# a1q123456/image_stitching

Measured on AMD Instinct MI355X. Metric: 4K frames stitched/sec, higher is better.
Workload: dtype u8

## Files before the change

image_stitching_amd/csrc/orb.hip:

```cpp
#include "common.h"
#include "dev_math.h"
#include <algorithm>
#include <cmath>
#include <mutex>
#include <unordered_map>

#define ORB_MAX_LEVELS 16
#define ORB_BORDER 32

namespace {

struct LevelDesc {
    int w, h;
    int pp;
    int sp;
    size_t pad_off;
    size_t map_off;
    float scale;
    int nfeat;
    int n2;
    int tiles_x, tiles_y, tile_off;
    int cap1, cand_off;
    int cap2, fin_off;
    int tab_off;
};

struct Levels {
    int n;
    int fast_t, patch, half_patch, edge;
    LevelDesc d[ORB_MAX_LEVELS];
};

struct Work {
    uint8_t *pad, *blur, *score, *nms;
    int* hist;
    int* thr;
    int* tile_cnt;
    uint32_t* surv_xy;
    uint8_t* surv_sc;
    int* cnt1;
    int* cnt2;
    int* flags;
    uint32_t* cand_xy;
    float* cand_resp;
    uint32_t* fin_xy;
    float* fin_resp;
    int* tab;
    int* umax;
    int8_t* pattern;
};

constexpr int ORB_BATCH = 16;
struct OrbIO {
    const uint8_t* src[ORB_BATCH];
    size_t sstride[ORB_BATCH];
    int aligned[ORB_BATCH];
    MisKeyPoint* kps[ORB_BATCH];
    uint32_t* lxy[ORB_BATCH];
    int* n_dev[ORB_BATCH];
    uint8_t* desc[ORB_BATCH];
// ... 157 lines not shown
    if ((px & 3) == 0) *reinterpret_cast<unsigned*>(p + ro + px) = v;
    else
#pragma unroll
        for (int k = 0; k < 4; k++) p[ro + px + k] = (uint8_t)(v >> (8 * k));
}

__device__ __forceinline__ bool fast_pretest(const uint8_t* p, int pp, int t) {
    const int v = p[0], hi = v + t, lo = v - t;
    const int c0 = p[3 * pp], c4 = p[3], c8 = p[-3 * pp], c12 = p[-3];
    unsigned br = (c0 > hi) | ((c4 > hi) << 2) | ((c8 > hi) << 4) | ((c12 > hi) << 6);
    unsigned dk = (c0 < lo) | ((c4 < lo) << 2) | ((c8 < lo) << 4) | ((c12 < lo) << 6);
    const unsigned adj_b = br & ((br >> 2) | (br << 6)), adj_d = dk & ((dk >> 2) | (dk << 6));
    if (!((adj_b | adj_d) & 0x55)) return false;
    const int c2 = p[2 * pp + 2], c6 = p[-2 * pp + 2], c10 = p[-2 * pp - 2], c14 = p[2 * pp - 2];
    br |= ((c2 > hi) << 1) | ((c6 > hi) << 3) | ((c10 > hi) << 5) | ((c14 > hi) << 7);
    dk |= ((c2 < lo) << 1) | ((c6 < lo) << 3) | ((c10 < lo) << 5) | ((c14 < lo) << 7);
    const unsigned b2 = br | (br << 8), d2 = dk | (dk << 8);
    const unsigned rb = b2 & (b2 >> 1) & (b2 >> 2) & (b2 >> 3), rd = d2 & (d2 >> 1) & (d2 >> 2) & (d2 >> 3);
    return ((rb | rd) & 0xff) != 0;
}
__device__ __forceinline__ int fast_score_full(const uint8_t* p, int pp, int t) {
    const int v = p[0];
    int d[16];
    d[0] = v - p[3 * pp]; d[1] = v - p[3 * pp + 1]; d[2] = v - p[2 * pp + 2]; d[3] = v - p[pp + 3];
    d[4] = v - p[3]; d[5] = v - p[-pp + 3]; d[6] = v - p[-2 * pp + 2]; d[7] = v - p[-3 * pp + 1];
    d[8] = v - p[-3 * pp]; d[9] = v - p[-3 * pp - 1]; d[10] = v - p[-2 * pp - 2]; d[11] = v - p[-pp - 3];
    d[12] = v - p[-3]; d[13] = v - p[pp - 3]; d[14] = v - p[2 * pp - 2]; d[15] = v - p[3 * pp - 1];
    int n3[16], x3[16];
#pragma unroll
    for (int i = 0; i < 16; i++) {
        n3[i] = min(min(d[i], d[(i + 1) & 15]), d[(i + 2) & 15]);
        x3[i] = max(max(d[i], d[(i + 1) & 15]), d[(i + 2) & 15]);
    }
    int A = -512, Bm = 512;
#pragma unroll
    for (int i = 0; i < 16; i++) {
        A = max(A, min(min(n3[i], n3[(i + 3) & 15]), n3[(i + 6) & 15]));
        Bm = min(Bm, max(max(x3[i], x3[(i + 3) & 15]), x3[(i + 6) & 15]));
    }
    const int best = max(A, -Bm);
    return best > t ? best - 1 : 0;
}
__device__ __forceinline__ int fast_score_px(const uint8_t* p, int pp, int t) { return fast_pretest(p, pp, t) ? fast_score_full(p, pp, t) : 0; }

#ifndef MIS_FT_ROWS
#define MIS_FT_ROWS 64
#endif
constexpr int FT_COLS = 64, FT_ROWS = MIS_FT_ROWS, FG_PITCH = 96, FG_COL0 = 15, HIST_COPIES = 8;
constexpr int FT_WR = (FT_ROWS + 2 + 3) / 4;
constexpr int FT_SLOTS = FT_COLS * FT_ROWS / 4;
#ifdef MIS_ORB_STATS
__device__ unsigned long long g_orb_stats[8];
#endif
__global__ __launch_bounds__(256) void fast_nms_kernel(Levels L, const uint8_t* pad, int* hist, int* tile_cnt, uint32_t* surv_xy, uint8_t* surv_sc, size_t ws) {
    __shared__ __attribute__((aligned(16))) uint8_t g[(FT_ROWS + 10) * FG_PITCH];
    __shared__ __attribute__((aligned(16))) uint8_t sc[(FT_ROWS + 2) * (FT_COLS + 4)];
    __shared__ int lh[256];
    __shared__ int lcount;
    __shared__ uint32_t lxy[FT_SLOTS];
    __shared__ uint8_t lsc[FT_SLOTS];
    __shared__ unsigned short queue[(FT_ROWS + 2) * (FT_COLS + 2)];
    __shared__ int qcount;
    const int fz = blockIdx.z / L.n, lz = blockIdx.z - fz * L.n;
    const LevelDesc& d = L.d[lz];
    const int x0 = blockIdx.x * FT_COLS, y0 = blockIdx.y * FT_ROWS, t = threadIdx.x;
    if (x0 >= d.w || y0 >= d.h) return;
    WS_OFF(pad, fz, ws); WS_OFF(hist, fz, ws); WS_OFF(tile_cnt, fz, ws); WS_OFF(surv_xy, fz, ws); WS_OFF(surv_sc, fz, ws);
    lh[t] = 0;
    if (t == 0) { lcount = 0; qcount = 0; }
    {
        const int ph = d.h + 2 * ORB_BORDER;
        const uint8_t* src = pad + d.pad_off;
        const int px0 = x0 - 16 + ORB_BORDER, py0 = y0 - 4 + ORB_BORDER;
        for (int i = t; i < (FT_ROWS + 8) * (FG_PITCH / 16); i += 256) {
            const int r = i / (FG_PITCH / 16), c = i - r * (FG_PITCH / 16);
            const int py = min(py0 + r, ph - 1);
            int px = px0 + 16 * c;
            if (px + 15 >= d.pp) px = d.pp - 16;
            reinterpret_cast<uint4*>(g)[i] = *reinterpret_cast<const uint4*>(src + (size_t)py * d.pp + px);
        }
    }
    __syncthreads();
    const int SP = FT_COLS + 4;
    for (int i = t; i < (FT_ROWS + 2) * SP / 4; i += 256) reinterpret_cast<unsigned*>(sc)[i] = 0u;
    {
        const int wv = __builtin_amdgcn_readfirstlane(t >> 6), lane = t & 63;
        const unsigned ft = (unsigned)L.fast_t;
        const int r0 = FT_WR * wv;
        bool pass[FT_WR + 1];
        unsigned long long ball[FT_WR + 1];
        int total = 0;
        {
            const uint8_t* colp = g + r0 * FG_PITCH + (lane + FG_COL0);
            unsigned col[FT_WR + 6];
#pragma unroll
            for (int j = 0; j < FT_WR + 6; j++) col[j] = colp[j * FG_PITCH];
            const int x = x0 - 1 + lane;
            const bool xin = x >= 3 && x < d.w - 3;
            const uint8_t* rowp = g + (r0 + 3) * FG_PITCH + (lane + FG_COL0 - 3);
#pragma unroll
            for (int k = 0; k < FT_WR; k++) {
                const int r = r0 + k, y = y0 - 1 + r;
                const bool rowok = r < FT_ROWS + 2 && y >= 3 && y < d.h - 3;
                const unsigned v = col[k + 3];
                const unsigned dv = max(__builtin_amdgcn_sad_u8(col[k + 6], v, 0u), __builtin_amdgcn_sad_u8(col[k], v, 0u));
                const unsigned dh = max(__builtin_amdgcn_sad_u8(rowp[k * FG_PITCH + 6], v, 0u), __builtin_amdgcn_sad_u8(rowp[k * FG_PITCH], v, 0u));
                pass[k] = rowok & xin & (min(dv, dh) > ft);
                ball[k] = __ballot(pass[k]);
                total += __popcll(ball[k]);
            }
        }
        {
            const int k = lane >> 1, cc = FT_COLS + (lane & 1), r = r0 + k, y = y0 - 1 + r, x = x0 - 1 + cc;
            bool ps = false;
            if (lane < 2 * FT_WR && r < FT_ROWS + 2) {
                const uint8_t* pp = g + (r + 3) * FG_PITCH + (cc + FG_COL0);
// ... 16 lines not shown
                const int r = k < FT_WR ? r0 + k : r0 + (lane >> 1), c = k < FT_WR ? lane : FT_COLS + (lane & 1);
                queue[base + __popcll(ball[k] & below)] = (unsigned short)(r * (FT_COLS + 2) + c);
            }
            base += __popcll(ball[k]);
        }
    }
    __syncthreads();
    for (int q = t; q < qcount; q += 256) {
        const int i = queue[q], r = i / (FT_COLS + 2), c = i - r * (FT_COLS + 2);
        const int fsv = fast_score_full(g + (r + 3) * FG_PITCH + (c + FG_COL0), FG_PITCH, L.fast_t);
        sc[r * SP + c] = (uint8_t)fsv;
#ifdef MIS_ORB_STATS
        if (fsv) atomicAdd(&g_orb_stats[3], 1ull);
#endif
    }
    __syncthreads();
    {
        const int nq = qcount;
        for (int q0 = 0; q0 < nq; q0 += 256) {
            const int q = q0 + t;
            bool keep = false;
            int x = 0, y = 0, v = 0;
            if (q < nq) {
                const int i = queue[q], r = i / (FT_COLS + 2), c = i - r * (FT_COLS + 2);
                const uint8_t* s_ = sc + r * SP + c;
                v = s_[0];
                x = x0 - 1 + c; y = y0 - 1 + r;
                keep = v && r >= 1 && r <= FT_ROWS && c >= 1 && c <= FT_COLS && x >= L.edge && x < d.w - L.edge && y >= L.edge && y < d.h - L.edge &&
                       v > s_[-1] && v > s_[1] && v > s_[-SP - 1] && v > s_[-SP] && v > s_[-SP + 1] && v > s_[SP - 1] && v > s_[SP] && v > s_[SP + 1];
            }
            const unsigned long long m = __ballot(keep);
            int base = 0;
            if ((t & 63) == 0 && m) base = atomicAdd(&lcount, __popcll(m));
            base = __shfl(base, 0);
            if (keep) {
                const int j = base + __popcll(m & ((1ull << (t & 63)) - 1ull));
                lxy[j] = (uint32_t)x | ((uint32_t)y << 16); lsc[j] = (uint8_t)v;
            }
        }
    }
    __syncthreads();
    const int n = lcount;
    const int tile = d.tile_off + blockIdx.y * d.tiles_x + blockIdx.x;
    if (t == 0) tile_cnt[tile] = n;
    if (n == 0) return;
    for (int j = t; j < n; j += 256) {
        atomicAdd(&lh[lsc[j]], 1);
        surv_xy[(size_t)tile * FT_SLOTS + j] = lxy[j]; surv_sc[(size_t)tile * FT_SLOTS + j] = lsc[j];
    }
    __syncthreads();
    if (lh[t]) atomicAdd(&hist[((lz * HIST_COPIES) + ((blockIdx.x + blockIdx.y) & (HIST_COPIES - 1))) * 256 + t], lh[t]);
}

__global__ __launch_bounds__(256) void fast_cut_kernel(Levels L, const int* hist, int* thr, int* flags, size_t ws) {
    __shared__ int suf[256];
    __shared__ int s_thr;
    const int l = blockIdx.x, t = threadIdx.x;
    WS_OFF(hist, blockIdx.y, ws); WS_OFF(thr, blockIdx.y, ws); WS_OFF(flags, blockIdx.y, ws);
    const LevelDesc& d = L.d[l];
    int hsum = 0;
    for (int c = 0; c < HIST_COPIES; c++) hsum += hist[(l * HIST_COPIES + c) * 256 + t];
    suf[t] = t ? hsum : 0;
    __syncthreads();
    for (int o = 1; o < 256; o <<= 1) {
        int add = t + o < 256 ? suf[t + o] : 0;
        __syncthreads();
        suf[t] += add;
        __syncthreads();
    }
    if (t == 0) s_thr = d.n2 == 0 ? 256 : 1;
    __syncthreads();
    if (d.n2 > 0 && suf[1] > d.n2 && t >= 1 && suf[t] >= d.n2 && (t == 255 || suf[t + 1] < d.n2)) s_thr = t;
    __syncthreads();
    if (t == 0) {
        thr[l] = s_thr;
        if (s_thr < 256 && suf[s_thr] > d.cap1) atomicOr(&flags[0], 1);
    }
}

constexpr int CT_TILES = 16;
__global__ __launch_bounds__(256) void compact_kernel(Levels L, const int* tile_cnt, const uint32_t* surv_xy, const uint8_t* surv_sc, const int* thr,
                                                      int* cnt1, uint32_t* cand_xy, float* cand_resp, size_t ws) {
    __shared__ int s_cnt[CT_TILES], s_off[CT_TILES];
    __shared__ int s_base;
    const int l = blockIdx.y, t = threadIdx.x, lane = t & 63, wave = t >> 6;
    WS_OFF(tile_cnt, blockIdx.z, ws); WS_OFF(surv_xy, blockIdx.z, ws); WS_OFF(surv_sc, blockIdx.z, ws); WS_OFF(thr, blockIdx.z, ws);
    WS_OFF(cnt1, blockIdx.z, ws); WS_OFF(cand_xy, blockIdx.z, ws); WS_OFF(cand_resp, blockIdx.z, ws);
    const LevelDesc& d = L.d[l];
    const int ntiles = d.tiles_x * d.tiles_y, first = blockIdx.x * CT_TILES;
    if (first >= ntiles) return;
    const int th = thr[l];
    for (int k = 0; k < CT_TILES / 4; k++) {
        const int slot = wave * (CT_TILES / 4) + k, til = first + slot;
        int cnt = 0;
        if (til < ntiles) {
            const int tile = d.tile_off + til, n = tile_cnt[tile];
            for (int j0 = 0; j0 < n; j0 += 64) {
                const int j = j0 + lane;
                const int v = j < n ? surv_sc[(size_t)tile * FT_SLOTS + j] : 0;
                cnt += __popcll(__ballot(v >= th && v > 0));
            }
        }
        if (lane == 0) s_cnt[slot] = cnt;
    }
    __syncthreads();
    if (t == 0) {
        int tot = 0;
        for (int k = 0; k < CT_TILES; k++) { s_off[k] = tot; tot += s_cnt[k]; }
        s_base = tot ? atomicAdd(&cnt1[l], tot) : 0;
    }
    __syncthreads();
    for (int k = 0; k < CT_TILES / 4; k++) {
        const int slot = wave * (CT_TILES / 4) + k, til = first + slot;
        if (til >= ntiles || s_cnt[slot] == 0) continue;
        const int tile = d.tile_off + til, n = tile_cnt[tile];
        int run = s_base + s_off[slot];
        for (int j0 = 0; j0 < n; j0 += 64) {
            const int j = j0 + lane;
            const int v = j < n ? surv_sc[(size_t)tile * FT_SLOTS + j] : 0;
            const bool keep = v >= th && v > 0;
            const unsigned long long m = __ballot(keep);
            if (keep) {
                const int i = run + __popcll(m & ((1ull << lane) - 1ull));
                if (i < d.cap1) { cand_xy[d.cand_off + i] = surv_xy[(size_t)tile * FT_SLOTS + j]; cand_resp[d.cand_off + i] = (float)v; }
            }
            run += __popcll(m);
        }
    }
}

__global__ void nms_raster_kernel(LevelDesc d, const int* tile_cnt, const uint32_t* surv_xy, const uint8_t* surv_sc, uint8_t* nms) {
    const int ntiles = d.tiles_x * d.tiles_y;
    for (int tl = blockIdx.x; tl < ntiles; tl += gridDim.x) {
        const int tile = d.tile_off + tl, n = tile_cnt[tile];
        for (int j = threadIdx.x; j < n; j += blockDim.x) {
            uint32_t xy = surv_xy[(size_t)tile * FT_SLOTS + j];
            nms[d.map_off + (size_t)(xy >> 16) * d.sp + (xy & 0xffff)] = surv_sc[(size_t)tile * FT_SLOTS + j];
        }
    }
}

__global__ __launch_bounds__(256) void harris_kernel(Levels L, const uint8_t* pad, const int* cnt1, const uint32_t* cand_xy, float* cand_resp, size_t ws) {
    const LevelDesc& d = L.d[blockIdx.y];
    WS_OFF(pad, blockIdx.z, ws); WS_OFF(cnt1, blockIdx.z, ws); WS_OFF(cand_xy, blockIdx.z, ws); WS_OFF(cand_resp, blockIdx.z, ws);
    int i = blockIdx.x * 256 + threadIdx.x;
    int n = min(cnt1[blockIdx.y], d.cap1);
    if (i >= n) return;
    uint32_t xy = cand_xy[d.cand_off + i];
    int x = xy & 0xffff, y = xy >> 16;
    const int pp = d.pp;
    const uint8_t* q0 = pad + d.pad_off + (size_t)(y + ORB_BORDER - 4) * pp + (x + ORB_BORDER - 4);
    const unsigned sh = (unsigned)((uintptr_t)q0 & 3u);
    const uint8_t* a0 = q0 - sh;
    int px[9][9];
#pragma unroll
    for (int r = 0; r < 9; r++) {
        const unsigned* row = reinterpret_cast<const unsigned*>(a0 + (size_t)r * pp);
        const unsigned d0 = row[0], d1 = row[1], d2 = row[2];
        const unsigned w0 = __builtin_amdgcn_alignbyte(d1, d0, sh), w1 = __builtin_amdgcn_alignbyte(d2, d1, sh), w2 = __builtin_amdgcn_alignbyte(0u, d2, sh);
#pragma unroll
        for (int k = 0; k < 4; k++) { px[r][k] = (int)((w0 >> (8 * k)) & 255u); px[r][4 + k] = (int)((w1 >> (8 * k)) & 255u); }
        px[r][8] = (int)(w2 & 255u);
    }
    int a = 0, b = 0, c = 0;
#pragma unroll
    for (int by = 0; by < 7; by++)
#pragma unroll
        for (int bx = 0; bx < 7; bx++) {
            const int Ix = (px[by + 1][bx + 2] - px[by + 1][bx]) * 2 + (px[by][bx + 2] - px[by][bx]) + (px[by + 2][bx + 2] - px[by + 2][bx]);
            const int Iy = (px[by + 2][bx + 1] - px[by][bx + 1]) * 2 + (px[by + 2][bx] - px[by][bx]) + (px[by + 2][bx + 2] - px[by][bx + 2]);
            a += Ix * Ix; b += Iy * Iy; c += Ix * Iy;
        }
    const float scale = 1.f / ((1 << 2) * 7 * 255.f);
    const float scale_sq_sq = scale * scale * scale * scale;
    float fa = (float)a, fb = (float)b, fc = (float)c;
    float s1 = fa * fb, s2 = fc * fc;
    float s3 = 0.04f * (fa + fb);
    s3 = s3 * (fa + fb);
    cand_resp[d.cand_off + i] = ((s1 - s2) - s3) * scale_sq_sq;
}

__device__ __forceinline__ uint32_t fkey(float f) {
    uint32_t u = __float_as_uint(f);
    return (u & 0x80000000u) ? ~u : (u | 0x80000000u);
}

__global__ __launch_bounds__(1024) void select_rank_kernel(Levels L, const int* cnt1, const uint32_t* cand_xy, const float* cand_resp,
                                                            int* cnt2, uint32_t* fin_xy, float* fin_resp, int* flags, int use_harris, size_t ws) {
    WS_OFF(cnt1, blockIdx.y, ws); WS_OFF(cand_xy, blockIdx.y, ws); WS_OFF(cand_resp, blockIdx.y, ws); WS_OFF(cnt2, blockIdx.y, ws);
    WS_OFF(fin_xy, blockIdx.y, ws); WS_OFF(fin_resp, blockIdx.y, ws); WS_OFF(flags, blockIdx.y, ws);
    __shared__ int hist[256];
    __shared__ uint32_t s_prefix, s_mask;
    __shared__ int s_k, s_m;
    __shared__ uint32_t kkey[4096], kxy[4096];
    const int l = blockIdx.x, t = threadIdx.x;
    const LevelDesc& d = L.d[l];
    const int n = min(cnt1[l], d.cap1);
    const uint32_t* xy = cand_xy + d.cand_off;
    const float* rs = cand_resp + d.cand_off;
    const int N = d.nfeat;
    if (N == 0) { if (t == 0) cnt2[l] = 0; return; }
    if (n <= 4096) {
        int P = 1;
        while (P < n) P <<= 1;
        for (int i = t; i < P; i += 1024) {
            if (i < n) { kkey[i] = fkey(rs[i]); kxy[i] = xy[i]; }
            else { kkey[i] = 0; kxy[i] = 0xffffffffu; }
        }
        __syncthreads();
        for (int k = 2; k <= P; k <<= 1)
            for (int j = k >> 1; j > 0; j >>= 1) {
                for (int i = t; i < P; i += 1024) {
                    const int ixj = i ^ j;
                    if (ixj > i) {
                        const uint32_t ka = kkey[i], kb = kkey[ixj], pa = kxy[i], pb = kxy[ixj];
                        const bool a_first = ka > kb || (ka == kb && pa < pb);
                        const bool descending_block = (i & k) == 0;
                        if (a_first != descending_block) { kkey[i] = kb; kkey[ixj] = ka; kxy[i] = pb; kxy[ixj] = pa; }
                    }
                }
                __syncthreads();
            }
        const uint32_t cutk = (use_harris && n > N) ? kkey[N - 1] : 0u;
        if (t == 0) s_m = 0;
        __syncthreads();
        for (int i = t; i < n; i += 1024)
            if (kkey[i] >= cutk && (i == n - 1 || kkey[i + 1] < cutk)) s_m = i + 1;
        __syncthreads();
        const int m = s_m;
        if (m > d.cap2) { if (t == 0) { atomicOr(&flags[0], 2); cnt2[l] = 0; } return; }
        for (int i = t; i < m; i += 1024) {
            fin_xy[d.fin_off + i] = kxy[i];
            const uint32_t ki = kkey[i], uu = (ki & 0x80000000u) ? (ki & 0x7fffffffu) : ~ki;
            fin_resp[d.fin_off + i] = __uint_as_float(uu);
        }
        if (t == 0) cnt2[l] = m;
        return;
    }
    uint32_t cut = 0;
    if (use_harris && n > N) {
        if (t == 0) { s_prefix = 0; s_mask = 0; s_k = N; }
        __syncthreads();
        for (int shift = 24; shift >= 0; shift -= 8) {
            if (t < 256) hist[t] = 0;
            __syncthreads();
            uint32_t prefix = s_prefix, mask = s_mask;
            for (int i = t; i < n; i += 1024) {
                uint32_t k = fkey(rs[i]);
// ... 266 lines not shown
        for (int j = 0; j < 7; j++) {
            const unsigned d0 = q[j * (DD_PITCH / 4)], d1 = q[j * (DD_PITCH / 4) + 1], d2 = q[j * (DD_PITCH / 4) + 2];
            const unsigned lo = __builtin_amdgcn_alignbit(d1, d0, sh), hi = __builtin_amdgcn_alignbit(d2, d1, sh);
            const unsigned hs = __builtin_amdgcn_udot4(lo, 0x38302212u, __builtin_amdgcn_udot4(hi, 0x00122230u, 0u, false), false);
            acc += (unsigned)kq[j] * hs;
            if (j == 3) centre = lo >> 24;
        }
        return inside ? (int)((acc + (1u << 15)) >> 16) : (int)centre;
    };
    int val = 0;
#ifndef DD_UNROLL
#define DD_UNROLL 1
#endif
#pragma unroll DD_UNROLL
    for (int bit = 0; bit < 4; bit++) {
        float x0 = (float)pat[4 * bit], y0 = (float)pat[4 * bit + 1], x1 = (float)pat[4 * bit + 2], y1 = (float)pat[4 * bit + 3];
        int ix0 = mis_round_f(x0 * ca - y0 * sa), iy0 = mis_round_f(x0 * sa + y0 * ca);
        int ix1 = mis_round_f(x1 * ca - y1 * sa), iy1 = mis_round_f(x1 * sa + y1 * ca);
        const int t0 = blurred(ix0, iy0), t1 = blurred(ix1, iy1);
        val |= (t0 < t1) << (bit + 4 * h);
    }
    val |= __shfl_xor(val, 32);
    if (h == 0) desc[(size_t)i * 32 + b] = (uint8_t)val;
}

constexpr int ORB_GATHER_MAX = 96;
struct GatherPtrs { const int* p[ORB_GATHER_MAX]; };
__global__ void gather_ints_kernel(GatherPtrs g, int n, int* __restrict__ out) {
    const int i = blockIdx.x * blockDim.x + threadIdx.x;
    if (i < n) out[i] = *g.p[i];
}

}

struct MisOrb {
    MisContext* ctx = nullptr;
    void (*enqueued_cb)(void*) = nullptr;
    void* enqueued_user = nullptr;
    MisOrbParams p;
    int max_w = 0, max_h = 0;
    int cur_w = 0, cur_h = 0;
    Levels L;
    Work w;
    size_t ws_stride = 0;
    int ws_frames = 0;
    int umax_host[64] = {0};
    int8_t pattern_host[1024] = {0};
    void* mem = nullptr;
    size_t pad_bytes = 0, map_bytes = 0;
    int cand_total = 0, fin_total = 0, tab_total = 0, surv_total = 0, out_cap = 0;
    std::vector<int> tab_host;
    int* host_counts = nullptr;
    bool direct_describe = false;
};

namespace {

void linear_exact_coeffs(int dlen, int slen, int* ofs, int* m1) {
    double inv = (double)dlen / (double)slen, scale = 1.0 / inv;
    for (int i = 0; i < dlen; i++) {
        double v = ((double)i + 0.5) * scale - 0.5;
        int iv = (int)floor(v);
        if (iv < 0) { ofs[i] = 0; m1[i] = 0; }
        else if (iv >= slen - 1) { ofs[i] = slen - 1; m1[i] = 0; }
        else { ofs[i] = iv; m1[i] = (int)lrint((v - (double)iv) * 256.0); }
    }
}

constexpr int ORB_MAX_LEVEL_FEATURES = 2048 - 128;

inline float level_scale(const MisOrbParams& p, int l) { return (float)pow((double)p.scale_factor, (double)l); }
inline int level_dim(int len, float sc) { return (int)lrint((double)((float)len / sc)); }

void level_budgets(const MisOrbParams& p, int* nfeat) {
    float factor = (float)(1.0 / (double)p.scale_factor);
    float nd = (float)p.nfeatures * (1 - factor) / (1 - (float)pow((double)factor, (double)p.nlevels));
    int sum = 0;
    for (int l = 0; l < p.nlevels - 1; l++) { nfeat[l] = (int)lrintf(nd); sum += nfeat[l]; nd *= factor; }
    nfeat[p.nlevels - 1] = std::max(p.nfeatures - sum, 0);
}

int check_level_sizes(MisContext* ctx, const MisOrbParams& p, int w, int h) {
    for (int l = 0; l < p.nlevels; l++) {
        const float sc = level_scale(p, l);
        MIS_CHECK(ctx, level_dim(w, sc) >= 1 && level_dim(h, sc) >= 1, MIS_E_UNSUPPORTED,
                  "ORB level %d of a %dx%d frame is empty (scale_factor %g, nlevels %d)", l, w, h, (double)p.scale_factor, p.nlevels);
    }
    return MIS_OK;
}

void plan_levels(MisOrb* o, int w, int h) {
    Levels& L = o->L;
    const MisOrbParams& p = o->p;
    L.n = p.nlevels; L.fast_t = p.fast_threshold; L.patch = p.patch_size; L.half_patch = p.patch_size / 2; L.edge = p.edge_threshold;
    size_t pad_off = 0, map_off = 0;
    int cand_off = 0, fin_off = 0, tab_off = 0, surv_off = 0;
    int nfeat[ORB_MAX_LEVELS];
    level_budgets(p, nfeat);
    for (int l = 0; l < L.n; l++) {
        LevelDesc& d = L.d[l];
        float sc = level_scale(p, l);
        d.scale = sc;
        d.w = level_dim(w, sc);
        d.h = level_dim(h, sc);
        d.pp = (int)mis_align_up((size_t)d.w + 2 * ORB_BORDER, 64);
        d.sp = (int)mis_align_up((size_t)d.w, 64);
// ... 7 lines not shown
        d.cap2 = std::min(d.nfeat + 128, 2048);
        d.cand_off = cand_off; cand_off += d.cap1;
        d.fin_off = fin_off; fin_off += d.cap2;
        d.tab_off = tab_off; tab_off += (2 * ((d.w + 3) & ~3) + 2 * d.h + 3) & ~3;
    }
    o->pad_bytes = pad_off; o->map_bytes = map_off; o->cand_total = cand_off; o->fin_total = fin_off; o->tab_total = tab_off; o->surv_total = surv_off;
    o->tab_host.assign(tab_off, 0);
    for (int l = 1; l < L.n; l++) {
        int* t = o->tab_host.data() + L.d[l].tab_off;
        const int dw4 = (L.d[l].w + 3) & ~3;
        linear_exact_coeffs(L.d[l].w, L.d[l - 1].w, t, t + dw4);
        linear_exact_coeffs(L.d[l].h, L.d[l - 1].h, t + 2 * dw4, t + 2 * dw4 + L.d[l].h);
    }
}

int upload_tables(MisOrb* o) {
    MisContext* ctx = o->ctx;
    if (o->tab_total)
        MIS_HIP(ctx, hipMemcpyAsync(o->w.tab, o->tab_host.data(), sizeof(int) * o->tab_total, hipMemcpyHostToDevice, ctx->stream));
    MIS_HIP(ctx, hipStreamSynchronize(ctx->stream));
    return MIS_OK;
}

std::mutex g_feat_mutex;
std::unordered_map<void*, size_t> g_feat_sizes;

int alloc_features(MisContext* ctx, int cap, int desc_cols, int desc_dtype, MisFeatures* f) {
    size_t kb = mis_align_up(sizeof(MisKeyPoint) * (size_t)cap, 256), db = mis_align_up((size_t)cap * desc_cols * mis_dtype_size(desc_dtype), 256);
    size_t lb = mis_align_up(sizeof(uint32_t) * (size_t)cap, 256);
    void* mem = nullptr;
    size_t got = 0;
    int rc = mis_pool_alloc(ctx, kb + db + lb + 256, &mem, &got);
    if (rc != MIS_OK) return rc;
    f->keypoints = (MisKeyPoint*)mem;
    f->descriptors = (uint8_t*)mem + kb;
    f->desc_cols = desc_cols; f->desc_dtype = desc_dtype;
    f->owner_ = mem;
    f->n = 0;
    std::lock_guard<std::mutex> lock(g_feat_mutex);
    g_feat_sizes[mem] = got;
    return MIS_OK;
}

inline uint32_t* feat_lxy(const MisFeatures* f, int cap) {
    size_t kb = mis_align_up(sizeof(MisKeyPoint) * (size_t)cap, 256), db = mis_align_up((size_t)cap * f->desc_cols * mis_dtype_size(f->desc_dtype), 256);
    return (uint32_t*)((uint8_t*)f->owner_ + kb + db);
}
inline int* feat_count(const MisFeatures* f, int cap) {
    size_t kb = mis_align_up(sizeof(MisKeyPoint) * (size_t)cap, 256), db = mis_align_up((size_t)cap * f->desc_cols * mis_dtype_size(f->desc_dtype), 256);
    size_t lb = mis_align_up(sizeof(uint32_t) * (size_t)cap, 256);
    return (int*)((uint8_t*)f->owner_ + kb + db + lb);
}

int enqueue_detect_group(MisOrb* o, const DevView* img, int w, int h, MisFeatures* out, int ng) {
    MisContext* ctx = o->ctx;
    const Levels& L = o->L;
    const Work& W = o->w;
    hipStream_t st = ctx->stream;
    const LevelDesc& d0 = L.d[0];
    const size_t ws = o->ws_stride;
    const unsigned nf = (unsigned)ng;
    OrbIO io;
    for (int k = 0; k < ORB_BATCH; k++) {
        const int q = k < ng ? k : 0;
        io.src[k] = (const uint8_t*)img[q].data; io.sstride[k] = img[q].stride;
        io.aligned[k] = (img[q].stride % 4 == 0) && ((uintptr_t)img[q].data % 4 == 0);
        io.kps[k] = out[q].keypoints; io.lxy[k] = feat_lxy(&out[q], o->out_cap); io.n_dev[k] = feat_count(&out[q], o->out_cap);
        io.desc[k] = (uint8_t*)out[q].descriptors;
    }
    MIS_HIP(ctx, hipMemset2DAsync(W.hist, ws ? ws : sizeof(int) * (256 * HIST_COPIES * ORB_MAX_LEVELS + 4 * ORB_MAX_LEVELS), 0,
                                  sizeof(int) * (256 * HIST_COPIES * ORB_MAX_LEVELS + 4 * ORB_MAX_LEVELS), nf, st));
    hipLaunchKernelGGL(gray_kernel, dim3((w + 1023) / 1024, (h + GRAY_ROWS - 1) / GRAY_ROWS, nf), dim3(256), 0, st, io, w, h, W.pad + d0.pad_off, d0.pp, ws);
    for (int l = 1; l < L.n; l++) {
        const LevelDesc &s = L.d[l - 1], &d = L.d[l];
        hipLaunchKernelGGL(resize_kernel, dim3((d.w + 255) / 256, (d.h + 4 * RS_ROWS - 1) / (4 * RS_ROWS), nf), dim3(256), 0, st, W.pad + s.pad_off, s.w, s.h, s.pp, W.pad + d.pad_off, d.w,
                           d.h, d.pp, W.tab + d.tab_off, ws);
    }
    const int pw0 = d0.w + 2 * ORB_BORDER, ph0 = d0.h + 2 * ORB_BORDER;
    hipLaunchKernelGGL((border_kernel<true>), dim3((d0.h * 16 + 255) / 256, 1, L.n * nf), dim3(256), 0, st, L, W.pad, ws);
    hipLaunchKernelGGL((border_kernel<false>), dim3((pw0 + 1023) / 1024, 2 * ORB_BORDER / 4, L.n * nf), dim3(256), 0, st, L, W.pad, ws);
    dim3 gmap((d0.w + FT_COLS - 1) / FT_COLS, (d0.h + FT_ROWS - 1) / FT_ROWS, L.n * nf);
    hipLaunchKernelGGL(fast_nms_kernel, gmap, dim3(256), 0, st, L, W.pad, W.hist, W.tile_cnt, W.surv_xy, W.surv_sc, ws);
    hipLaunchKernelGGL(fast_cut_kernel, dim3(L.n, nf), dim3(256), 0, st, L, W.hist, W.thr, W.flags, ws);
    hipLaunchKernelGGL(compact_kernel, dim3((d0.tiles_x * d0.tiles_y + CT_TILES - 1) / CT_TILES, L.n, nf), dim3(256), 0, st, L, W.tile_cnt, W.surv_xy, W.surv_sc, W.thr, W.cnt1,
                       W.cand_xy, W.cand_resp, ws);
    const int use_harris = o->p.score_type == 0;
    if (use_harris)
        hipLaunchKernelGGL(harris_kernel, dim3((L.d[0].cap1 + 255) / 256, L.n, nf), dim3(256), 0, st, L, W.pad, W.cnt1, W.cand_xy, W.cand_resp, ws);
    hipLaunchKernelGGL(select_rank_kernel, dim3(L.n, nf), dim3(1024), 0, st, L, W.cnt1, W.cand_xy, W.cand_resp, W.cnt2, W.fin_xy, W.fin_resp, W.flags,
                       use_harris, ws);
    hipLaunchKernelGGL(assemble_angle_kernel, dim3((o->out_cap + 3) / 4, nf), dim3(256), 0, st, L, W.pad, W.cnt2, W.fin_xy, W.fin_resp, W.umax, io, o->out_cap, ws, o->direct_describe ? 0 : 1);
    if (o->direct_describe) {
        UMax16 um16;
        for (int v = 0; v < 16; v++) um16.v[v] = o->umax_host[v];
        hipLaunchKernelGGL(describe_direct_kernel, dim3((o->out_cap + 3) / 4, nf), dim3(256), 0, st, L, W.pad, io, W.pattern, W.umax, um16, ws);
    } else {
        for (int k = 0; k < ng; k++) {
            hipLaunchKernelGGL(blur_kernel, dim3((pw0 + 63) / 64, (ph0 + 31) / 32, L.n), dim3(256), 0, st, L, W.pad + k * ws, W.blur + k * ws);
            hipLaunchKernelGGL(describe_kernel, dim3((o->out_cap + 7) / 8), dim3(256), 0, st, L, W.blur + k * ws, out[k].keypoints, io.lxy[k], io.n_dev[k], W.pattern,
                               (uint8_t*)out[k].descriptors);
        }
    }
    MIS_HIP(ctx, hipGetLastError());
    return MIS_OK;
}

int check_image(MisOrb* o, const MisImage* bgr) {
    MisContext* ctx = o->ctx;
    MIS_CHECK(ctx, bgr && bgr->data, MIS_E_INVALID, "null image");
    MIS_CHECK(ctx, bgr->dtype == MIS_U8 && bgr->channels == 3, MIS_E_UNSUPPORTED, "ORB input must be 8UC3 (BGR)");
    MIS_CHECK(ctx, bgr->width <= o->max_w && bgr->height <= o->max_h && bgr->width >= 64 && bgr->height >= 64, MIS_E_INVALID,
              "image %dx%d outside the finder's range (64x64 .. %dx%d)", bgr->width, bgr->height, o->max_w, o->max_h);
    return MIS_OK;
}

int replan_if_needed(MisOrb* o, int w, int h) {
    if (w == o->cur_w && h == o->cur_h) return MIS_OK;
    const int rc = check_level_sizes(o->ctx, o->p, w, h);
    if (rc != MIS_OK) return rc;
    MIS_HIP(o->ctx, hipStreamSynchronize(o->ctx->stream));
    plan_levels(o, w, h);
    o->cur_w = w; o->cur_h = h;
    return upload_tables(o);
}

int orb_alloc_workspace(MisOrb* o, int frames) {
    MisContext* ctx = o->ctx;
    size_t off = 0;
    auto carve = [&](size_t bytes) { size_t o_ = off; off += mis_align_up(bytes, 256); return o_; };
    const bool frame_blur = !o->direct_describe;
    size_t o_pad = carve(o->pad_bytes), o_blur = frame_blur ? carve(o->pad_bytes) : 0;
    size_t o_hist = carve(sizeof(int) * (256 * HIST_COPIES * ORB_MAX_LEVELS + 4 * ORB_MAX_LEVELS)), o_flags = carve(256);
    size_t o_sxy = carve(sizeof(uint32_t) * FT_SLOTS * (size_t)o->surv_total), o_ssc = carve(FT_SLOTS * (size_t)o->surv_total), o_tc = carve(sizeof(int) * (size_t)o->surv_total);
    size_t o_cxy = carve(sizeof(uint32_t) * o->cand_total), o_cr = carve(sizeof(float) * o->cand_total);
    size_t o_fxy = carve(sizeof(uint32_t) * o->fin_total), o_fr = carve(sizeof(float) * o->fin_total);
    size_t o_tab = carve(sizeof(int) * (o->tab_total + 4)), o_umax = carve(sizeof(int) * 64), o_pat = carve(1024);
    const size_t tail = mis_align_up(o->map_bytes, 256) + (frame_blur ? 0 : mis_align_up(o->pad_bytes, 256));
    void* mem = nullptr;
    if (hipMalloc(&mem, off * (size_t)frames + tail) != hipSuccess) return mis_set_error(ctx, MIS_E_NOMEM, "hipMalloc of %zu bytes failed", off * (size_t)frames + tail);
    o->mem = mem; o->ws_stride = off; o->ws_frames = frames;
    uint8_t* m = (uint8_t*)o->mem;
    uint8_t* shared = m + off * (size_t)frames;
    Work& W = o->w;
    W.pad = m + o_pad; W.nms = shared; W.blur = frame_blur ? m + o_blur : shared + mis_align_up(o->map_bytes, 256); W.score = nullptr;
    W.hist = (int*)(m + o_hist); W.thr = W.hist + 256 * HIST_COPIES * ORB_MAX_LEVELS; W.cnt1 = W.thr + ORB_MAX_LEVELS; W.cnt2 = W.cnt1 + ORB_MAX_LEVELS;
    W.surv_xy = (uint32_t*)(m + o_sxy); W.surv_sc = m + o_ssc; W.tile_cnt = (int*)(m + o_tc);
    W.flags = (int*)(m + o_flags);
    W.cand_xy = (uint32_t*)(m + o_cxy); W.cand_resp = (float*)(m + o_cr); W.fin_xy = (uint32_t*)(m + o_fxy); W.fin_resp = (float*)(m + o_fr);
    W.tab = (int*)(m + o_tab); W.umax = (int*)(m + o_umax); W.pattern = (int8_t*)(m + o_pat);
    return MIS_OK;
}

int orb_init_workspace(MisOrb* o) {
    MisContext* ctx = o->ctx;
    const Work& W = o->w;
    MIS_HIP(ctx, hipMemcpyAsync(W.umax, o->umax_host, sizeof(o->umax_host), hipMemcpyHostToDevice, ctx->stream));
    MIS_HIP(ctx, hipMemcpyAsync(W.pattern, o->pattern_host, sizeof(o->pattern_host), hipMemcpyHostToDevice, ctx->stream));
    MIS_HIP(ctx, hipMemset2DAsync(W.flags, o->ws_stride, 0, 256, (size_t)o->ws_frames, ctx->stream));
    MIS_HIP(ctx, hipStreamSynchronize(ctx->stream));
    return upload_tables(o);
}

int orb_ensure_frames(MisOrb* o, int frames) {
    frames = std::min(frames, ORB_BATCH);
    if (o->ws_frames >= frames) return MIS_OK;
    MisContext* ctx = o->ctx;
    MIS_HIP(ctx, hipStreamSynchronize(ctx->stream));
    void* old = o->mem;
    const Work oldw = o->w;
    const size_t olds = o->ws_stride;
    const int oldf = o->ws_frames;
    int rc = MIS_E_NOMEM;
    for (int f = frames; f > oldf; f = std::max(oldf, f / 2)) {
        if ((rc = orb_alloc_workspace(o, f)) == MIS_OK) break;
    }
    if (rc != MIS_OK) {
        o->mem = old; o->w = oldw; o->ws_stride = olds; o->ws_frames = oldf;
        return oldf >= 1 ? MIS_OK : rc;
    }
    if (old) MIS_HIP(ctx, hipFree(old));
    return orb_init_workspace(o);
}

}

int mis_feat_block_alloc(MisContext* ctx, size_t bytes, void** out, MisContext* errs) {
    size_t got = 0;
    const int rc = mis_pool_alloc(ctx, bytes, out, &got, errs);
    if (rc != MIS_OK) return rc;
    std::lock_guard<std::mutex> lock(g_feat_mutex);
    g_feat_sizes[*out] = got;
    return MIS_OK;
}


extern "C" void mis_orb_default_params(MisOrbParams* p) {
    if (p) *p = MisOrbParams{4000, 1.2f, 8, 1, 0, 2, 0, 40, 20};
}

extern "C" int mis_orb_create(MisContext* ctx, const MisOrbParams* p, int max_w, int max_h, MisOrb** out) {
    if (!ctx || !out) return MIS_E_INVALID;
    MIS_CHECK(ctx, p, MIS_E_INVALID, "null params");
    MIS_CHECK(ctx, p->nlevels >= 1 && p->nlevels <= ORB_MAX_LEVELS && p->first_level == 0 && p->wta_k == 2 && p->patch_size >= 2 &&
                       p->patch_size <= 40 && p->nfeatures >= 1 && p->scale_factor > 1.f && (p->score_type == 0 || p->score_type == 1) &&
                       p->edge_threshold >= 0 && p->fast_threshold >= 1 && p->fast_threshold < 255,
              MIS_E_UNSUPPORTED, "unsupported ORB parameters (need first_level 0, wta_k 2, patch <= 40, nlevels <= 16)");
    MIS_CHECK(ctx, p->patch_size != 31, MIS_E_UNSUPPORTED, "ORB patch_size 31 (OpenCV's fixed bit_pattern_31_) is not supported");
    {
        int nfeat[ORB_MAX_LEVELS];
        level_budgets(*p, nfeat);
        for (int l = 0; l < p->nlevels; l++)
            MIS_CHECK(ctx, nfeat[l] <= ORB_MAX_LEVEL_FEATURES, MIS_E_UNSUPPORTED,
                      "ORB nfeatures %d gives level %d a budget of %d keypoints (at most %d per level)", p->nfeatures, l, nfeat[l], ORB_MAX_LEVEL_FEATURES);
    }
    MIS_CHECK(ctx, max_w >= 64 && max_h >= 64 && max_w <= 32767 && max_h <= 32767, MIS_E_INVALID, "bad maximum size");
    if (int rc = check_level_sizes(ctx, *p, max_w, max_h)) return rc;
    MIS_HIP(ctx, hipSetDevice(ctx->device));
    MisOrb* o = new MisOrb();
    o->ctx = ctx; o->p = *p; o->max_w = max_w; o->max_h = max_h;
    plan_levels(o, max_w, max_h);
    o->out_cap = o->fin_total;
    int umax[64] = {0};
    {
        int hp = p->patch_size / 2, v, v0;
        int vmax = (int)floor((double)((float)hp * sqrtf(2.f) / 2 + 1));
        int vmin = (int)ceil((double)((float)hp * sqrtf(2.f) / 2));
        for (v = 0; v <= vmax; ++v) umax[v] = (int)lrint(sqrt((double)hp * hp - (double)v * v));
        for (v = hp, v0 = 0; v >= vmin; --v) {
            while (umax[v0] == umax[v0 + 1]) ++v0;
            umax[v] = v0;
            ++v0;
        }
    }
    int8_t pat[1024];
    {
        uint64_t state = 0x34985739u;
        auto next = [&]() { state = (uint64_t)(uint32_t)state * 4164903690u + (uint32_t)(state >> 32); return (uint32_t)state; };
        int hp = p->patch_size / 2;
        for (int i = 0; i < 1024; i++) pat[i] = (int8_t)(int)(next() % (uint32_t)(2 * hp + 1) + (uint32_t)(-hp));
    }
    {
        int max_sq = 0;
        for (int i = 0; i < 512; i++) max_sq = std::max(max_sq, (int)pat[2 * i] * pat[2 * i] + (int)pat[2 * i + 1] * pat[2 * i + 1]);
        const int reach = (int)floor(sqrt((double)max_sq) + 0.5);
        o->direct_describe = reach <= DD_R && 3 + ORB_BORDER >= DD_P;
    }
    int rc0 = orb_alloc_workspace(o, 1);
    if (rc0 != MIS_OK) { delete o; return rc0; }
    memcpy(o->umax_host, umax, sizeof(umax));
    memcpy(o->pattern_host, pat, sizeof(pat));
    o->cur_w = max_w; o->cur_h = max_h;
    int rc = orb_init_workspace(o);
    if (rc != MIS_OK) { hipFree(o->mem); delete o; return rc; }
    *out = o;
    return MIS_OK;
}

extern "C" int mis_orb_destroy(MisOrb* o) {
    if (!o) return MIS_OK;
    hipSetDevice(o->ctx->device);
    hipStreamSynchronize(o->ctx->stream);
    if (o->mem) hipFree(o->mem);
    if (o->host_counts) hipHostFree(o->host_counts);
    delete o;
    return MIS_OK;
}


extern "C" int mis_orb_detect_batch(MisOrb* o, const MisImage* imgs, int n, MisFeatures* out) {
    if (!o) return MIS_E_INVALID;
    MisContext* ctx = o->ctx;
    MIS_CHECK(ctx, imgs && out && n >= 1, MIS_E_INVALID, "null argument");
    MIS_HIP(ctx, hipSetDevice(ctx->device));
    int rc;
    for (int i = 0; i < n; i++) {
        if ((rc = check_image(o, &imgs[i])) != MIS_OK) return rc;
        MIS_CHECK(ctx, imgs[i].width == imgs[0].width && imgs[i].height == imgs[0].height, MIS_E_INVALID, "batch frames must share one size");
    }
    if ((rc = replan_if_needed(o, imgs[0].width, imgs[0].height)) != MIS_OK) return rc;
    if ((rc = orb_ensure_frames(o, n)) != MIS_OK) return rc;
    std::vector<DevView> dimg(n);
    for (int i = 0; i < n; i++) memset(&out[i], 0, sizeof(MisFeatures));
    auto fail = [&](int code) {
        hipStreamSynchronize(ctx->stream);
        for (int i = 0; i < n; i++)
            if (out[i].keypoints || out[i].descriptors) mis_features_free(ctx, &out[i]);
        return code;
    };
    for (int i = 0; i < n; i++) {
        out[i].img_idx = i; out[i].img_w = imgs[i].width; out[i].img_h = imgs[i].height;
        if ((rc = alloc_features(ctx, o->out_cap, 32, MIS_U8, &out[i])) != MIS_OK) return fail(rc);
        if ((rc = dimg[i].read(ctx, &imgs[i])) != MIS_OK) return fail(rc);
    }
    const bool trace = getenv("MIS_ORB_TRACE") != nullptr;
    const auto t_enq0 = std::chrono::steady_clock::now();
    for (int g0 = 0; g0 < n; g0 += o->ws_frames) {
        const int ng = std::min(o->ws_frames, n - g0);
        if ((rc = enqueue_detect_group(o, &dimg[g0], imgs[0].width, imgs[0].height, &out[g0], ng)) != MIS_OK) return fail(rc);
    }
    if (trace) fprintf(stderr, "orb batch: %d frames enqueued in %.0f us\n", n, (double)std::chrono::duration_cast<std::chrono::microseconds>(std::chrono::steady_clock::now() - t_enq0).count());
    if (o->enqueued_cb) {
        void (*cb)(void*) = o->enqueued_cb;
        void* user = o->enqueued_user;
        o->enqueued_cb = nullptr; o->enqueued_user = nullptr;
        cb(user);
        MIS_HIP(ctx, hipSetDevice(ctx->device));
    }
    std::vector<int> counts(n);
    const int nl = o->ws_frames;
    std::vector<int> ws_flags(nl, 0);
    if (!o->host_counts) MIS_HIP(ctx, hipHostMalloc((void**)&o->host_counts, sizeof(int) * ORB_GATHER_MAX, hipHostMallocMapped));
    for (int i0 = 0; i0 < n + nl; i0 += ORB_GATHER_MAX) {
        const int m = std::min(ORB_GATHER_MAX, n + nl - i0);
        GatherPtrs gp;
        for (int k = 0; k < m; k++)
            gp.p[k] = i0 + k < n ? feat_count(&out[i0 + k], o->out_cap) : (const int*)((const char*)o->w.flags + (size_t)(i0 + k - n) * o->ws_stride);
// ... 113 lines not shown
```

Before: 3365.

## Overlap FAST detection with pyramid resize using an auxiliary stream

```diff
diff --git a/image_stitching_amd/csrc/orb.hip b/image_stitching_amd/csrc/orb.hip
--- a/image_stitching_amd/csrc/orb.hip
+++ b/image_stitching_amd/csrc/orb.hip
@@ -6,6 +6,7 @@
 #include <unordered_map>
 
 #define ORB_MAX_LEVELS 16
+#define ORB_MAX_GROUPS 2
 #define ORB_BORDER 32
 
 namespace {
@@ -269,7 +270,7 @@
 #ifdef MIS_ORB_STATS
 __device__ unsigned long long g_orb_stats[8];
 #endif
-__global__ __launch_bounds__(256) void fast_nms_kernel(Levels L, const uint8_t* pad, int* hist, int* tile_cnt, uint32_t* surv_xy, uint8_t* surv_sc, size_t ws) {
+__global__ __launch_bounds__(256) void fast_nms_kernel(Levels L, int l0, int nl, const uint8_t* pad, int* hist, int* tile_cnt, uint32_t* surv_xy, uint8_t* surv_sc, size_t ws) {
     __shared__ __attribute__((aligned(16))) uint8_t g[(FT_ROWS + 10) * FG_PITCH];
     __shared__ __attribute__((aligned(16))) uint8_t sc[(FT_ROWS + 2) * (FT_COLS + 4)];
     __shared__ int lh[256];
@@ -278,7 +279,7 @@
     __shared__ uint8_t lsc[FT_SLOTS];
     __shared__ unsigned short queue[(FT_ROWS + 2) * (FT_COLS + 2)];
     __shared__ int qcount;
-    const int fz = blockIdx.z / L.n, lz = blockIdx.z - fz * L.n;
+    const int fz = blockIdx.z / nl, lz = l0 + (blockIdx.z - fz * nl);
     const LevelDesc& d = L.d[lz];
     const int x0 = blockIdx.x * FT_COLS, y0 = blockIdx.y * FT_ROWS, t = threadIdx.x;
     if (x0 >= d.w || y0 >= d.h) return;
@@ -401,10 +402,10 @@
     if (lh[t]) atomicAdd(&hist[((lz * HIST_COPIES) + ((blockIdx.x + blockIdx.y) & (HIST_COPIES - 1))) * 256 + t], lh[t]);
 }
 
-__global__ __launch_bounds__(256) void fast_cut_kernel(Levels L, const int* hist, int* thr, int* flags, size_t ws) {
+__global__ __launch_bounds__(256) void fast_cut_kernel(Levels L, int l0, const int* hist, int* thr, int* flags, size_t ws) {
     __shared__ int suf[256];
     __shared__ int s_thr;
-    const int l = blockIdx.x, t = threadIdx.x;
+    const int l = l0 + blockIdx.x, t = threadIdx.x;
     WS_OFF(hist, blockIdx.y, ws); WS_OFF(thr, blockIdx.y, ws); WS_OFF(flags, blockIdx.y, ws);
     const LevelDesc& d = L.d[l];
     int hsum = 0;
@@ -428,11 +429,11 @@
 }
 
 constexpr int CT_TILES = 16;
-__global__ __launch_bounds__(256) void compact_kernel(Levels L, const int* tile_cnt, const uint32_t* surv_xy, const uint8_t* surv_sc, const int* thr,
+__global__ __launch_bounds__(256) void compact_kernel(Levels L, int l0, const int* tile_cnt, const uint32_t* surv_xy, const uint8_t* surv_sc, const int* thr,
                                                       int* cnt1, uint32_t* cand_xy, float* cand_resp, size_t ws) {
     __shared__ int s_cnt[CT_TILES], s_off[CT_TILES];
     __shared__ int s_base;
-    const int l = blockIdx.y, t = threadIdx.x, lane = t & 63, wave = t >> 6;
+    const int l = l0 + blockIdx.y, t = threadIdx.x, lane = t & 63, wave = t >> 6;
     WS_OFF(tile_cnt, blockIdx.z, ws); WS_OFF(surv_xy, blockIdx.z, ws); WS_OFF(surv_sc, blockIdx.z, ws); WS_OFF(thr, blockIdx.z, ws);
     WS_OFF(cnt1, blockIdx.z, ws); WS_OFF(cand_xy, blockIdx.z, ws); WS_OFF(cand_resp, blockIdx.z, ws);
     const LevelDesc& d = L.d[l];
@@ -489,11 +490,12 @@
     }
 }
 
-__global__ __launch_bounds__(256) void harris_kernel(Levels L, const uint8_t* pad, const int* cnt1, const uint32_t* cand_xy, float* cand_resp, size_t ws) {
-    const LevelDesc& d = L.d[blockIdx.y];
+__global__ __launch_bounds__(256) void harris_kernel(Levels L, int l0, const uint8_t* pad, const int* cnt1, const uint32_t* cand_xy, float* cand_resp, size_t ws) {
+    const int l = l0 + blockIdx.y;
+    const LevelDesc& d = L.d[l];
     WS_OFF(pad, blockIdx.z, ws); WS_OFF(cnt1, blockIdx.z, ws); WS_OFF(cand_xy, blockIdx.z, ws); WS_OFF(cand_resp, blockIdx.z, ws);
     int i = blockIdx.x * 256 + threadIdx.x;
-    int n = min(cnt1[blockIdx.y], d.cap1);
+    int n = min(cnt1[l], d.cap1);
     if (i >= n) return;
     uint32_t xy = cand_xy[d.cand_off + i];
     int x = xy & 0xffff, y = xy >> 16;
@@ -534,7 +536,7 @@
     return (u & 0x80000000u) ? ~u : (u | 0x80000000u);
 }
 
-__global__ __launch_bounds__(1024) void select_rank_kernel(Levels L, const int* cnt1, const uint32_t* cand_xy, const float* cand_resp,
+__global__ __launch_bounds__(1024) void select_rank_kernel(Levels L, int l0, const int* cnt1, const uint32_t* cand_xy, const float* cand_resp,
                                                             int* cnt2, uint32_t* fin_xy, float* fin_resp, int* flags, int use_harris, size_t ws) {
     WS_OFF(cnt1, blockIdx.y, ws); WS_OFF(cand_xy, blockIdx.y, ws); WS_OFF(cand_resp, blockIdx.y, ws); WS_OFF(cnt2, blockIdx.y, ws);
     WS_OFF(fin_xy, blockIdx.y, ws); WS_OFF(fin_resp, blockIdx.y, ws); WS_OFF(flags, blockIdx.y, ws);
@@ -542,7 +544,7 @@
     __shared__ uint32_t s_prefix, s_mask;
     __shared__ int s_k, s_m;
     __shared__ uint32_t kkey[4096], kxy[4096];
-    const int l = blockIdx.x, t = threadIdx.x;
+    const int l = l0 + blockIdx.x, t = threadIdx.x;
     const LevelDesc& d = L.d[l];
     const int n = min(cnt1[l], d.cap1);
     const uint32_t* xy = cand_xy + d.cand_off;
@@ -915,6 +917,10 @@
     std::vector<int> tab_host;
     int* host_counts = nullptr;
     bool direct_describe = false;
+    hipStream_t aux = nullptr;
+    hipEvent_t ev_level[ORB_MAX_LEVELS] = {nullptr};
+    hipEvent_t ev_fast[ORB_MAX_GROUPS] = {nullptr};
+    hipEvent_t ev_join = nullptr;
 };
 
 namespace {
@@ -1028,11 +1034,21 @@
     return (int*)((uint8_t*)f->owner_ + kb + db + lb);
 }
 
-int enqueue_detect_group(MisOrb* o, const DevView* img, int w, int h, MisFeatures* out, int ng) {
+struct LevelGroup { int l0, nl; };
+int level_groups(int nlevels, bool two_streams, LevelGroup* g) {
+    if (!two_streams || nlevels < 2) { g[0] = {0, nlevels}; return 1; }
+    g[0] = {0, 1}; g[1] = {1, nlevels - 1};
+    return 2;
+}
+
+constexpr size_t ORB_TWO_STREAM_MIN_PIXELS = 40000000;
+
+int enqueue_detect_graph(MisOrb* o, const DevView* img, int w, int h, MisFeatures* out, int ng, hipStream_t sb) {
     MisContext* ctx = o->ctx;
     const Levels& L = o->L;
     const Work& W = o->w;
     hipStream_t st = ctx->stream;
+    const bool two = sb != st;
     const LevelDesc& d0 = L.d[0];
     const size_t ws = o->ws_stride;
     const unsigned nf = (unsigned)ng;
@@ -1044,27 +1060,49 @@
         io.kps[k] = out[q].keypoints; io.lxy[k] = feat_lxy(&out[q], o->out_cap); io.n_dev[k] = feat_count(&out[q], o->out_cap);
         io.desc[k] = (uint8_t*)out[q].descriptors;
     }
+    LevelGroup grp[ORB_MAX_GROUPS];
+    const int ngrp = level_groups(L.n, two, grp);
     MIS_HIP(ctx, hipMemset2DAsync(W.hist, ws ? ws : sizeof(int) * (256 * HIST_COPIES * ORB_MAX_LEVELS + 4 * ORB_MAX_LEVELS), 0,
                                   sizeof(int) * (256 * HIST_COPIES * ORB_MAX_LEVELS + 4 * ORB_MAX_LEVELS), nf, st));
     hipLaunchKernelGGL(gray_kernel, dim3((w + 1023) / 1024, (h + GRAY_ROWS - 1) / GRAY_ROWS, nf), dim3(256), 0, st, io, w, h, W.pad + d0.pad_off, d0.pp, ws);
+    int gf = 0;
+    auto fast_upto = [&](int level) -> int {
+        for (; gf < ngrp && grp[gf].l0 + grp[gf].nl - 1 <= level; gf++) {
+            const LevelGroup& g = grp[gf];
+            const LevelDesc& dg = L.d[g.l0];
+            if (two) {
+                MIS_HIP(ctx, hipEventRecord(o->ev_level[level], st));
+                MIS_HIP(ctx, hipStreamWaitEvent(sb, o->ev_level[level], 0));
+            }
+            hipLaunchKernelGGL(fast_nms_kernel, dim3(dg.tiles_x, dg.tiles_y, g.nl * nf), dim3(256), 0, sb, L, g.l0, g.nl, W.pad, W.hist, W.tile_cnt, W.surv_xy, W.surv_sc, ws);
+            if (two) MIS_HIP(ctx, hipEventRecord(o->ev_fast[gf], sb));
+        }
+        return MIS_OK;
+    };
+    if (int rc = fast_upto(0)) return rc;
     for (int l = 1; l < L.n; l++) {
         const LevelDesc &s = L.d[l - 1], &d = L.d[l];
         hipLaunchKernelGGL(resize_kernel, dim3((d.w + 255) / 256, (d.h + 4 * RS_ROWS - 1) / (4 * RS_ROWS), nf), dim3(256), 0, st, W.pad + s.pad_off, s.w, s.h, s.pp, W.pad + d.pad_off, d.w,
                            d.h, d.pp, W.tab + d.tab_off, ws);
+        if (int rc = fast_upto(l)) return rc;
     }
     const int pw0 = d0.w + 2 * ORB_BORDER, ph0 = d0.h + 2 * ORB_BORDER;
     hipLaunchKernelGGL((border_kernel<true>), dim3((d0.h * 16 + 255) / 256, 1, L.n * nf), dim3(256), 0, st, L, W.pad, ws);
     hipLaunchKernelGGL((border_kernel<false>), dim3((pw0 + 1023) / 1024, 2 * ORB_BORDER / 4, L.n * nf), dim3(256), 0, st, L, W.pad, ws);
-    dim3 gmap((d0.w + FT_COLS - 1) / FT_COLS, (d0.h + FT_ROWS - 1) / FT_ROWS, L.n * nf);
-    hipLaunchKernelGGL(fast_nms_kernel, gmap, dim3(256), 0, st, L, W.pad, W.hist, W.tile_cnt, W.surv_xy, W.surv_sc, ws);
-    hipLaunchKernelGGL(fast_cut_kernel, dim3(L.n, nf), dim3(256), 0, st, L, W.hist, W.thr, W.flags, ws);
-    hipLaunchKernelGGL(compact_kernel, dim3((d0.tiles_x * d0.tiles_y + CT_TILES - 1) / CT_TILES, L.n, nf), dim3(256), 0, st, L, W.tile_cnt, W.surv_xy, W.surv_sc, W.thr, W.cnt1,
-                       W.cand_xy, W.cand_resp, ws);
     const int use_harris = o->p.score_type == 0;
-    if (use_harris)
-        hipLaunchKernelGGL(harris_kernel, dim3((L.d[0].cap1 + 255) / 256, L.n, nf), dim3(256), 0, st, L, W.pad, W.cnt1, W.cand_xy, W.cand_resp, ws);
-    hipLaunchKernelGGL(select_rank_kernel, dim3(L.n, nf), dim3(1024), 0, st, L, W.cnt1, W.cand_xy, W.cand_resp, W.cnt2, W.fin_xy, W.fin_resp, W.flags,
-                       use_harris, ws);
+    for (int k = 0; k < ngrp; k++) {
+        const LevelGroup& g = grp[k];
+        int cap1 = 0, ntiles = 0;
+        for (int l = g.l0; l < g.l0 + g.nl; l++) { cap1 = std::max(cap1, L.d[l].cap1); ntiles = std::max(ntiles, L.d[l].tiles_x * L.d[l].tiles_y); }
+        if (two) MIS_HIP(ctx, hipStreamWaitEvent(st, o->ev_fast[k], 0));
+        hipLaunchKernelGGL(fast_cut_kernel, dim3(g.nl, nf), dim3(256), 0, st, L, g.l0, W.hist, W.thr, W.flags, ws);
+        hipLaunchKernelGGL(compact_kernel, dim3((ntiles + CT_TILES - 1) / CT_TILES, g.nl, nf), dim3(256), 0, st, L, g.l0, W.tile_cnt, W.surv_xy, W.surv_sc, W.thr, W.cnt1,
+                           W.cand_xy, W.cand_resp, ws);
+        if (use_harris)
+            hipLaunchKernelGGL(harris_kernel, dim3((cap1 + 255) / 256, g.nl, nf), dim3(256), 0, st, L, g.l0, W.pad, W.cnt1, W.cand_xy, W.cand_resp, ws);
+        hipLaunchKernelGGL(select_rank_kernel, dim3(g.nl, nf), dim3(1024), 0, st, L, g.l0, W.cnt1, W.cand_xy, W.cand_resp, W.cnt2, W.fin_xy, W.fin_resp, W.flags,
+                           use_harris, ws);
+    }
     hipLaunchKernelGGL(assemble_angle_kernel, dim3((o->out_cap + 3) / 4, nf), dim3(256), 0, st, L, W.pad, W.cnt2, W.fin_xy, W.fin_resp, W.umax, io, o->out_cap, ws, o->direct_describe ? 0 : 1);
     if (o->direct_describe) {
         UMax16 um16;
@@ -1079,6 +1117,16 @@
     }
     MIS_HIP(ctx, hipGetLastError());
     return MIS_OK;
+}
+
+int enqueue_detect_group(MisOrb* o, const DevView* img, int w, int h, MisFeatures* out, int ng) {
+    const bool two = (size_t)ng * (size_t)w * (size_t)h >= ORB_TWO_STREAM_MIN_PIXELS;
+    const int rc = enqueue_detect_graph(o, img, w, h, out, ng, two ? o->aux : o->ctx->stream);
+    if (rc != MIS_OK && two) {
+        if (hipEventRecord(o->ev_join, o->aux) != hipSuccess || hipStreamWaitEvent(o->ctx->stream, o->ev_join, 0) != hipSuccess)
+            hipStreamSynchronize(o->aux);
+    }
+    return rc;
 }
 
 int check_image(MisOrb* o, const MisImage* bgr) {
@@ -1137,6 +1185,20 @@
     return upload_tables(o);
 }
 
+void orb_destroy_graph_objects(MisOrb* o) {
+    for (int l = 0; l < ORB_MAX_LEVELS; l++) if (o->ev_level[l]) { hipEventDestroy(o->ev_level[l]); o->ev_level[l] = nullptr; }
+    for (int g = 0; g < ORB_MAX_GROUPS; g++) if (o->ev_fast[g]) { hipEventDestroy(o->ev_fast[g]); o->ev_fast[g] = nullptr; }
+    if (o->ev_join) { hipEventDestroy(o->ev_join); o->ev_join = nullptr; }
+}
+int orb_create_graph_objects(MisOrb* o) {
+    MisContext* ctx = o->ctx;
+    if (int rc = mis_aux_stream(ctx, 0, &o->aux)) return rc;
+    for (int l = 0; l < o->p.nlevels; l++) MIS_HIP(ctx, hipEventCreateWithFlags(&o->ev_level[l], hipEventDisableTiming));
+    for (int g = 0; g < ORB_MAX_GROUPS; g++) MIS_HIP(ctx, hipEventCreateWithFlags(&o->ev_fast[g], hipEventDisableTiming));
+    MIS_HIP(ctx, hipEventCreateWithFlags(&o->ev_join, hipEventDisableTiming));
+    return MIS_OK;
+}
+
 int orb_ensure_frames(MisOrb* o, int frames) {
     frames = std::min(frames, ORB_BATCH);
     if (o->ws_frames >= frames) return MIS_OK;
@@ -1221,13 +1283,14 @@
         const int reach = (int)floor(sqrt((double)max_sq) + 0.5);
         o->direct_describe = reach <= DD_R && 3 + ORB_BORDER >= DD_P;
     }
-    int rc0 = orb_alloc_workspace(o, 1);
-    if (rc0 != MIS_OK) { delete o; return rc0; }
+    int rc0 = orb_create_graph_objects(o);
+    if (rc0 == MIS_OK) rc0 = orb_alloc_workspace(o, 1);
+    if (rc0 != MIS_OK) { orb_destroy_graph_objects(o); delete o; return rc0; }
     memcpy(o->umax_host, umax, sizeof(umax));
     memcpy(o->pattern_host, pat, sizeof(pat));
     o->cur_w = max_w; o->cur_h = max_h;
     int rc = orb_init_workspace(o);
-    if (rc != MIS_OK) { hipFree(o->mem); delete o; return rc; }
+    if (rc != MIS_OK) { hipFree(o->mem); orb_destroy_graph_objects(o); delete o; return rc; }
     *out = o;
     return MIS_OK;
 }
@@ -1236,8 +1299,10 @@
     if (!o) return MIS_OK;
     hipSetDevice(o->ctx->device);
     hipStreamSynchronize(o->ctx->stream);
+    if (o->aux) hipStreamSynchronize(o->aux);
     if (o->mem) hipFree(o->mem);
     if (o->host_counts) hipHostFree(o->host_counts);
+    orb_destroy_graph_objects(o);
     delete o;
     return MIS_OK;
 }
```

After: 3460 (median of 5 runs). 1.03x the previous value.
